# pedro-morgado/spatialaudiogen

Hardware: AMD Instinct MI355X
Metric: ambisonic seconds generated/sec (0.1 s windows, 224x448 video) (higher is better)
Workload: dtype f32 (fp32 in / out / accumulate; products on the 16-bit matrix cores with fp32-equivalent operand splits: two fp16 planes (3 products per multiply) for the ResNet trunk's 3x3 convs, whose operand ranges batch-norm bounds, three bf16 planes (6 products) elsewhere - measured against the fp64 oracle as

## Files before the change

spatialaudiogen_amd/csrc/conv3g.hip:

```cpp
#include "igemm3_common.h"

namespace sagen {

typedef _Float16 f16x8g __attribute__((ext_vector_type(8)));

constexpr int conv3g_wgs_per_cu(int BM, int BN, int KS, bool H2) {
    const int lds = 2 * KS * (BM + BN) * (H2 ? 64 : 96) + 512;
    return 3 * lds <= 160 * 1024 ? 3 : (2 * lds <= 160 * 1024 ? 2 : 1);
}

template <int BM, int BN, int WM, int WN, int KS, bool H2, int EPI = 0>
__global__ __launch_bounds__(256, conv3g_wgs_per_cu(BM, BN, KS, H2)) void conv3g_kernel(const IgemmDesc d_in) {
    IgemmDesc d = d_in;
    if (d.grp.G > 1) igemm_relocate(d, (int)blockIdx.z);
    constexpr int MT = WM / 32, NT = WN / 32;
    constexpr int WAVES_N = BN / WN, WAVES_M = BM / WM;
    static_assert(WAVES_N * WAVES_M == 4, "4 waves per workgroup");
    constexpr int NPL = H2 ? 2 : 3, SB = NPL * 32, UPS = NPL * 2;
    constexpr int NPR = H2 ? 3 : 6;
    constexpr int A_INST = BM * UPS / 64, B_INST = BN * UPS / 64;
    static_assert(BM * UPS % 64 == 0 && BN * UPS % 64 == 0, "operand images must be whole DMA instructions");
    constexpr int A_PW = (A_INST + 3) / 4, B_PW = (B_INST + 3) / 4;
    constexpr int A_BYTES = A_INST * 1024, B_BYTES = B_INST * 1024;
    constexpr int T_BYTES = A_BYTES + B_BYTES;
    constexpr int ST_BYTES = KS * T_BYTES;
    constexpr int SPT = A_PW + B_PW;
    constexpr int CNT = KS * SPT;
    constexpr int NM1 = NPR * MT * NT;
    constexpr int NMG = KS * NM1;
    static_assert(CNT <= NMG, "one DMA slot per MFMA slot at most");
    constexpr int NF = NPL * (MT + NT);
    constexpr int SMEM_BYTES = 2 * ST_BYTES;
    __shared__ __attribute__((aligned(16))) char smem[SMEM_BYTES];

    const int tid = threadIdx.x;
    const int lane = tid & 63;
    const int wave = __builtin_amdgcn_readfirstlane(tid >> 6);
    const int wm = wave / WAVES_N, wn = wave % WAVES_N;
    const int Wp = d.Win + 1;
    const int HinP = d.xp3_rows > 0 ? d.xp3_rows : d.Hin;
    const int nchunk = d.Cin >> 4;
    const int NKT = d.ntaps * nchunk;
    const int G = (NKT + KS - 1) / KS;
    const int nM = (d.M + BM - 1) / BM, nN = (d.N + BN - 1) / BN;

    const __amdgpu_buffer_rsrc_t x_rsrc = __builtin_amdgcn_make_buffer_rsrc((void*)d.xp3, 0, d.xp3_bytes, 0x00020000);
    const __amdgpu_buffer_rsrc_t w_rsrc = H2 ? __builtin_amdgcn_make_buffer_rsrc((void*)d.wh2, 0, d.wh2_bytes, 0x00020000)
                                             : __builtin_amdgcn_make_buffer_rsrc((void*)(d.w + (size_t)d.N * d.Kpad), 0, d.w_bytes / 2 * 3, 0x00020000);

    const int xcd = (blockIdx.x + blockIdx.z) & 7;
    const int per = (nM + 7) >> 3;
    const int t_run = blockIdx.x >> 3;
    const int my_tiles = max(min((xcd + 1) * per, nM) - xcd * per, 0) * nN;
    if (t_run >= my_tiles) return;
    const int tq = t_run / nN;
    const int m0 = (xcd * per + tq) * BM, n0 = (t_run - tq * nN) * BN;

    unsigned a_base[A_PW], a_bad[A_PW], a_cur[A_PW];
#pragma unroll
    for (int j = 0; j < A_PW; ++j) {
        const int inst = wave + 4 * j;
        const int U = inst * 64 + lane;
        const int slot = U / UPS, rem = U - UPS * slot;
        const int unit = H2 ? (rem ^ ((slot >> 2) & 3)) : ((rem & ~1) | ((rem & 1) ^ ((slot >> 3) & 1)));
        const int m = m0 + slot;
        a_base[j] = 0; a_bad[j] = 0xffffffffu;
        if (inst < A_INST && m < d.M) {
            const unsigned row = __umulhi((unsigned)m, d.p3_magic_wp);
            const int wo = m - (int)row * d.Wg;
            const unsigned b = __umulhi(row, d.p3_magic_h);
            const int ho = (int)row - (int)b * d.Hg;
            const int hi = (d.g_h0 + ho) * d.in_sh + d.tap_h0 - d.xp3_row0, wi = (d.g_w0 + wo) * d.in_sw + d.tap_w0;
            const int pix = ((int)b * HinP + hi) * Wp + wi;
            a_base[j] = (unsigned)(pix * SB + unit * 16);
            unsigned bad = 0;
            for (int th = 0; th * d.TW < d.ntaps; ++th) {
                const int hh = hi + th * d.tap_sh;
                if (hh < 0 || hh >= HinP) bad |= 1u << th;
            }
            a_bad[j] = bad;
        }
    }
    unsigned b_voff[B_PW];
#pragma unroll
    for (int j = 0; j < B_PW; ++j) {
        const int inst = wave + 4 * j;
        const int L = inst * 64 + lane;
        const int pl = L / (2 * BN), n = (L >> 1) % BN, half = L & 1;
        b_voff[j] = (inst < B_INST && n0 + n < d.N) ? (unsigned)((pl * d.N + n0 + n) * 32 + 16 * (half ^ ((n >> 3) & 1))) : OOB;
    }

    int q_th = 0, q_tw = 0, q_ch = 0, q_kt = 0;
    unsigned i_asoff = 0, i_bsoff = 0, i_dead = 0;
    char* i_tile = smem;
    auto begin_tile = [&](char* dst) {
        i_tile = dst;
        i_dead = q_kt >= NKT ? OOB : 0u;
        const unsigned tapd = (unsigned)((q_th * d.tap_sh * Wp + q_tw * d.tap_sw) * SB);
#pragma unroll
        for (int j = 0; j < A_PW; ++j) a_cur[j] = ((a_bad[j] >> q_th) & 1u) ? OOB : a_base[j] + tapd;
        i_asoff = (unsigned)q_ch * d.xp3_cstride;
        i_bsoff = (unsigned)q_kt * (unsigned)(d.N * SB);
        ++q_kt; ++q_ch;
        const int wrap_c = q_ch == nchunk ? 1 : 0;
        q_ch = wrap_c ? 0 : q_ch;
        q_tw += wrap_c;
        const int wrap_w = q_tw == d.TW ? 1 : 0;
        q_tw = wrap_w ? 0 : q_tw;
        q_th += wrap_w;
    };
    auto issue_one = [&](int s) {
        if (s < A_PW) {
            const int inst = wave + 4 * s;
            if (A_INST % 4 == 0 || inst < A_INST) dma16(x_rsrc, (float*)(i_tile + inst * 1024), a_cur[s] | i_dead, i_dead ? 0u : i_asoff);
        } else {
            const int j = s - A_PW;
            const int inst = wave + 4 * j;
            if (B_INST % 4 == 0 || inst < B_INST) dma16(w_rsrc, (float*)(i_tile + A_BYTES + inst * 1024), b_voff[j] | i_dead, i_dead ? 0u : i_bsoff);
        }
    };

    f32x16 acc[MT][NT];
#pragma unroll
    for (int i = 0; i < MT; ++i)
#pragma unroll
        for (int j = 0; j < NT; ++j)
#pragma unroll
            for (int e = 0; e < 16; ++e) acc[i][j][e] = 0.f;

    const int li = lane & 31, kk = lane >> 5;
    int a_foff[MT];
#pragma unroll
    for (int i = 0; i < MT; ++i) {
        const int sl = wm * WM + i * 32 + li;
        a_foff[i] = H2 ? sl * 64 + 16 * (kk ^ ((sl >> 2) & 3)) : sl * 96 + 16 * (kk ^ ((sl >> 3) & 1));
    }
    const int b_foff = A_BYTES + (wn * WN + li) * 32 + 16 * (kk ^ ((li >> 3) & 1));
    constexpr int TA[6] = {H2 ? 1 : 0, 0, H2 ? 0 : 1, 0, 2, 1}, TB[6] = {0, 1, 0, 2, 0, 1};

    int stage = 0;
#pragma unroll
    for (int ks = 0; ks < KS; ++ks) {
        begin_tile(smem + ks * T_BYTES);
#pragma unroll
        for (int s = SPT - 1; s >= 0; --s) issue_one(s);
    }

    auto group = [&](auto issue_tag) {
        constexpr bool ISSUE = decltype(issue_tag)::value;
        const char* st = smem + stage * ST_BYTES;
        char* const nst = smem + (stage ^ 1) * ST_BYTES;
        bf16x8 fq[2][NF];
        auto load_frag = [&](int buf, int ks, int f) {
            const int pl = f / (MT + NT), r = f - pl * (MT + NT);
            const char* tb = st + ks * T_BYTES;
            if (r < MT) fq[buf][f] = *reinterpret_cast<const bf16x8*>(tb + (H2 ? (a_foff[r] ^ (pl * 32)) : a_foff[r] + pl * 32));
            else fq[buf][f] = *reinterpret_cast<const bf16x8*>(tb + b_foff + pl * (BN * 32) + (r - MT) * 32 * 32);
        };
#pragma unroll
        for (int f = 0; f < NF; ++f) load_frag(0, 0, f);
#pragma unroll
        for (int ks = 0; ks < KS; ++ks) {
            const int cb = ks & 1;
#pragma unroll
            for (int tt = 0; tt < NPR; ++tt)
#pragma unroll
                for (int i = 0; i < MT; ++i)
#pragma unroll
                    for (int j = 0; j < NT; ++j) {
                        const int k = (tt * MT + i) * NT + j;
                        const int idx = ks * NM1 + k;
                        __builtin_amdgcn_sched_barrier(0);
                        if constexpr (H2)
                            acc[i][j] = __builtin_amdgcn_mfma_f32_32x32x16_f16(__builtin_bit_cast(f16x8g, fq[cb][TA[tt] * (MT + NT) + i]),
                                                                               __builtin_bit_cast(f16x8g, fq[cb][TB[tt] * (MT + NT) + MT + j]), acc[i][j], 0, 0, 0);
                        else
                            acc[i][j] = __builtin_amdgcn_mfma_f32_32x32x16_bf16(fq[cb][TA[tt] * (MT + NT) + i], fq[cb][TB[tt] * (MT + NT) + MT + j],
                                                                                acc[i][j], 0, 0, 0);
                        if (ks + 1 < KS) {
#pragma unroll
                            for (int f = 0; f < NF; ++f)
                                if (f * NM1 / NF == k) load_frag(cb ^ 1, ks + 1, f);
                        }
                        if (ISSUE && idx < CNT) {
                            const int tks = idx / SPT, s = idx - tks * SPT;
                            if (s == 0) begin_tile(nst + tks * T_BYTES);
                            issue_one(SPT - 1 - s);
                        }
                    }
        }
        __builtin_amdgcn_sched_barrier(0);
        stage ^= 1;
    };

    for (int it = 0; it + 1 < G; ++it) {
        asm volatile("s_waitcnt vmcnt(0)" ::: "memory");
        lds_barrier();
        group(std::true_type{});
    }
    asm volatile("s_waitcnt vmcnt(0)" ::: "memory");
    lds_barrier();
    group(std::false_type{});

    float osc = 1.f;
    if constexpr (H2) osc = d.h2_a_inv[0] * d.h2_w_inv[0];
    lds_barrier();
    if constexpr (EPI == 1) {
        if constexpr (H2) {
#pragma unroll
            for (int i = 0; i < MT; ++i)
#pragma unroll
                for (int j = 0; j < NT; ++j)
#pragma unroll
                    for (int e = 0; e < 16; ++e) acc[i][j][e] *= osc;
        }
        igemm_epilogue_maskmix<BM, BN, WM, WN, SMEM_BYTES / 4>(d, acc, reinterpret_cast<float*>(smem), m0, n0, tid);
        return;
    }
    {
        const int colb = n0 + wn * WN + li;
        const bool plain = d.bias == nullptr && !d.relu_out;
        const __amdgpu_buffer_rsrc_t y_rsrc = __builtin_amdgcn_make_buffer_rsrc((void*)d.y, 0, d.y_bytes, 0x00020000);
        const unsigned ldy4 = (unsigned)d.ldy * 4u;
        const int mrow = m0 + wm * WM + 4 * kk;
        const unsigned rbase = (unsigned)mrow * ldy4;
        float bias_j[NT], cs[NT], cq[NT];
        float amax = 0.f;
        unsigned col4[NT];
#pragma unroll
        for (int j = 0; j < NT; ++j) {
            const bool ok = colb + 32 * j < d.N;
            col4[j] = ok ? (unsigned)(colb + 32 * j) * 4u : OOB;
            bias_j[j] = (d.bias != nullptr && ok) ? d.bias[colb + 32 * j] : 0.f;
            cs[j] = 0.f; cq[j] = 0.f;
        }
        auto epilogue = [&](auto fast_tag) {
            constexpr bool FAST = decltype(fast_tag)::value;
#pragma unroll
            for (int i = 0; i < MT; ++i)
#pragma unroll
                for (int e = 0; e < 16; ++e) {
                    const int ro = i * 32 + (e & 3) + 8 * (e >> 2);
                    const bool ok = mrow + ro < d.M;
                    const float sc = ok ? osc : 0.f;
                    const unsigned roff = ok ? rbase + (unsigned)ro * ldy4 + (FAST ? (unsigned)(colb * 4) : 0u) : OOB;
#pragma unroll
                    for (int j = 0; j < NT; ++j) {
                        float v = acc[i][j][e] * sc;
                        if (FAST) {
                            cs[j] += v;
                            cq[j] = __builtin_fmaf(v, v, cq[j]);
                            __builtin_amdgcn_raw_buffer_store_b32(__builtin_bit_cast(unsigned, v), y_rsrc, roff, 128 * j, 0);
                        } else {
                            const unsigned off = ((roff | col4[j]) & OOB) ? OOB : roff + col4[j];
                            if (col4[j] & OOB) v = 0.f;
                            cs[j] += v;
                            cq[j] = __builtin_fmaf(v, v, cq[j]);
                            v += bias_j[j];
                            if (d.relu_out) v = fmaxf(v, 0.f);
                            amax = fmaxf(amax, (off & OOB) ? 0.f : fabsf(v));
                            __builtin_amdgcn_raw_buffer_store_b32(__builtin_bit_cast(unsigned, v), y_rsrc, off, 0, 0);
                        }
                    }
                }
        };
        if (plain && n0 + BN <= d.N && d.amax_out == nullptr) epilogue(std::true_type{});
        else epilogue(std::false_type{});
        if (d.amax_out != nullptr) igemm_publish_amax(d.amax_out, amax);
        if (d.stats != nullptr) {
            lds_barrier();
            float* const red = reinterpret_cast<float*>(smem);
            static_assert(WAVES_M * 2 * 2 * BN * 4 <= SMEM_BYTES, "statistics staging must fit the ring");
#pragma unroll
            for (int j = 0; j < NT; ++j) {
                red[((wm * 2 + kk) * 2 + 0) * BN + wn * WN + j * 32 + li] = cs[j];
                red[((wm * 2 + kk) * 2 + 1) * BN + wn * WN + j * 32 + li] = cq[j];
            }
            lds_barrier();
            for (int t = tid; t < 2 * BN; t += 256) {
                const int which = t / BN, col = t - which * BN;
                if (n0 + col < d.N) {
                    float sum = 0.f;
#pragma unroll
                    for (int g = 0; g < WAVES_M * 2; ++g) sum += red[(g * 2 + which) * BN + col];
                    atomicAdd(&d.stats[(long)which * d.N + n0 + col], (double)sum);
                }
            }
        }
    }
}

template <int BM, int BN, int WM, int WN, int KS, bool H2, int EPI = 0>
static int launch_conv3g(const IgemmDesc& d, hipStream_t s) {
    const int per = (cdiv(d.M, BM) + 7) / 8;
    const int grid = 8 * per * cdiv(d.N, BN);
    hipLaunchKernelGGL((conv3g_kernel<BM, BN, WM, WN, KS, H2, EPI>), dim3(grid, 1, d.grp.G), dim3(256), 0, s, d);
    SAGEN_LAUNCH_CHECK();
    return SAGEN_OK;
}

bool conv3g_ok(const IgemmDesc& d) {
    if (d.Cin % 16 || d.K != d.ntaps * d.Cin || d.Kpad != d.K) return false;
    if (d.ntaps < 1 || d.TW < 1 || d.ntaps % d.TW || d.ntaps / d.TW > 32) return false;
    if (d.in_scale != nullptr || d.bn_in.acc != nullptr) return false;
    if (d.mm_out != nullptr) {
        if (d.xp3_fmt != 1 || d.Cout != 32 || d.dsh * d.dsw <= 1 || d.Wg % 64 || (d.dsw * d.Cout) % 128 || d.splitk != 1 || !d.mm_coeffs) return false;
    } else {
        if (d.dsh * d.dsw != 1 || d.g_h0 != 0 || d.g_w0 != 0) return false;
        if (d.y_rstride != (long)d.Wg * d.ldy || (d.M > d.Hg * d.Wg && d.y_bstride != (long)d.Hg * d.Wg * d.ldy)) return false;
    }
    const int t_lo = std::min(0, (d.TW - 1) * d.tap_sw), t_hi = std::max(0, (d.TW - 1) * d.tap_sw);
    const int w_lo = d.g_w0 * d.in_sw + d.tap_w0 + t_lo, w_hi = (d.g_w0 + d.Wg - 1) * d.in_sw + d.tap_w0 + t_hi;
    return w_lo >= -1 && w_hi <= d.Win;
}

int conv3g_dispatch(const IgemmDesc& d_in, IgemmTile tile, hipStream_t s) {
    IgemmDesc d = d_in;
    if (!d.xp3 || d.p3_np <= 0) return fail(SAGEN_ERR_NULL, "conv3g: the P3 activation planes are missing");
    if (d.splitk != 1) return fail(SAGEN_ERR_UNSUPPORTED, "conv3g: no split-K");
    if (!conv3g_ok(d)) return fail(SAGEN_ERR_UNSUPPORTED, "conv3g: geometry not supported");
    if ((long)(d.M + 512) * d.Wg >= (1L << 32) || ((long)(d.M + 512) / d.Wg + 1) * d.Hg >= (1L << 32))
        return fail(SAGEN_ERR_UNSUPPORTED, "conv3g: too many pixels for 32-bit index arithmetic");
    if ((long)d.p3_np * 96 >= (1L << 31) || (long)d.xp3_cstride * (d.Cin / 16) >= (1L << 31) || d.xp3_bytes == 0)
        return fail(SAGEN_ERR_UNSUPPORTED, "conv3g: the activation planes exceed 2 GiB buffer addressing (use a smaller batch)");
    const bool mm = igemm_tile_traits(tile) & TF_FUSED_TAIL;
    if (mm != (d.mm_out != nullptr)) return fail(SAGEN_ERR_UNSUPPORTED, "conv3g: the fused decoder tail and the tile do not match");
    const bool h2 = igemm_tile_traits(tile) & TF_FP16X2;
    if (h2 != (d.xp3_fmt == 1)) return fail(SAGEN_ERR_UNSUPPORTED, "conv3g: the planes' format does not match the tile");
    if (h2 && (!d.wh2 || !d.h2_a_inv || !d.h2_w_inv)) return fail(SAGEN_ERR_NULL, "conv3g: the fp16x2 filter planes / scales are missing");
    if (!mm) {
        const long y_bytes = ((long)(d.M - 1) * d.ldy + d.N) * 4;
        if (y_bytes >= (1L << 31)) return fail(SAGEN_ERR_UNSUPPORTED, "conv3g: the output exceeds 2 GiB buffer addressing (use a smaller batch)");
        d.y_bytes = (unsigned)y_bytes;
    }
    d.p3_magic_wp = (unsigned)((1UL << 32) / (unsigned)d.Wg) + 1u;
    d.p3_magic_h = (unsigned)((1UL << 32) / (unsigned)d.Hg) + 1u;
#define SAGEN_TILE_HAS_P3G ,
#define SAGEN_TILE_HAS_P3GH ,
#define SAGEN_TILE_HAS_P3GH_MM ,
    switch (tile) {
        SAGEN_TILES(SAGEN_TILE_CASE)
        default: return fail(SAGEN_ERR_UNSUPPORTED, "conv3g: bad tile id %d", (int)tile);
    }
}

}
```

spatialaudiogen_amd/csrc/igemm_common.h:

```cpp
#pragma once
#include "kernels.h"
#include "h2_planes.h"

namespace sagen {

typedef float f32x16 __attribute__((ext_vector_type(16)));
constexpr int MAX_TAPS = 128;
constexpr unsigned OOB = 0x80000000u;
constexpr int MAX_BN_C = 512;

struct RowInfo {
    unsigned boff;
    unsigned nmlo, nmhi;
    int hrem, wrem;
    int pad;
    long rowoff;
};

__device__ __forceinline__ void dma16(__amdgpu_buffer_rsrc_t rsrc, float* lds, unsigned voff, unsigned soff) {
#if defined(__HIP_DEVICE_COMPILE__) && !defined(SAGEN_ABLATE_DMA)
    __builtin_amdgcn_raw_ptr_buffer_load_lds(rsrc, (__attribute__((address_space(3))) void*)lds, 16, voff, soff, 0, 0);
#endif
}

template <int N> __device__ __forceinline__ void wait_vmcnt() {
    if constexpr (N == 0) asm volatile("s_waitcnt vmcnt(0)" ::: "memory");
    else if constexpr (N == 1) asm volatile("s_waitcnt vmcnt(1)" ::: "memory");
    else if constexpr (N == 2) asm volatile("s_waitcnt vmcnt(2)" ::: "memory");
    else if constexpr (N == 3) asm volatile("s_waitcnt vmcnt(3)" ::: "memory");
    else if constexpr (N == 4) asm volatile("s_waitcnt vmcnt(4)" ::: "memory");
    else if constexpr (N == 5) asm volatile("s_waitcnt vmcnt(5)" ::: "memory");
    else if constexpr (N == 6) asm volatile("s_waitcnt vmcnt(6)" ::: "memory");
    else if constexpr (N == 7) asm volatile("s_waitcnt vmcnt(7)" ::: "memory");
    else if constexpr (N == 8) asm volatile("s_waitcnt vmcnt(8)" ::: "memory");
    else if constexpr (N == 9) asm volatile("s_waitcnt vmcnt(9)" ::: "memory");
    else asm volatile("s_waitcnt vmcnt(0)" ::: "memory");
}

__device__ __forceinline__ void lds_barrier() {
    asm volatile("s_waitcnt lgkmcnt(0)" ::: "memory");
    __builtin_amdgcn_s_barrier();
    asm volatile("" ::: "memory");
}


template <int BM>
__device__ __forceinline__ void igemm_setup(const IgemmDesc& d, int m0, int tid, bool uni, RowInfo* s_row, int* s_tapb,
                                            float (*s_bn)[MAX_BN_C]) {
    const int HgWg = d.Hg * d.Wg;
    if (!uni)
        for (int t = tid; t < d.ntaps; t += 256) {
            const int th = t / d.TW;
            s_tapb[t] = (((th * d.tap_sh + d.tap_h0) * d.Win + ((t - th * d.TW) * d.tap_sw + d.tap_w0)) * d.ldx) * 4;
        }
    for (int r = tid; r < BM; r += 256) {
        const int m = m0 + r;
        RowInfo ri;
        ri.boff = 0; ri.nmlo = 0xffffffffu; ri.nmhi = 0xffffffffu; ri.hrem = 0; ri.wrem = 0; ri.pad = 0; ri.rowoff = 0;
        if (m < d.M) {
            const int b = m / HgWg;
            const int rem = m - b * HgWg;
            const int ia = rem / d.Wg;
            const int a = d.g_h0 + ia, bb = d.g_w0 + (rem - ia * d.Wg);
            const int hi0 = a * d.in_sh, wi0 = bb * d.in_sw;
            ri.boff = (unsigned)(((long)b * d.x_bstride + ((long)hi0 * d.Win + wi0) * d.ldx) * 4);
            ri.rowoff = (long)b * d.y_bstride + (long)(a * d.dsh) * d.y_rstride + (long)(bb * d.dsw) * d.ldy;
            ri.hrem = d.Hlim - a * d.dsh;
            ri.wrem = d.Wlim - bb * d.dsw;
            if (d.no_bounds) {
                ri.nmlo = 0; ri.nmhi = 0;
            } else {
                unsigned lo = 0, hi = 0;
                for (int t = 0; t < d.ntaps; ++t) {
                    const int th = t / d.TW;
                    const int hh = hi0 + th * d.tap_sh + d.tap_h0, ww = wi0 + (t - th * d.TW) * d.tap_sw + d.tap_w0;
                    const unsigned bad = ((unsigned)hh < (unsigned)d.Hin && (unsigned)ww < (unsigned)d.Win) ? 0u : 1u;
                    if (t < 32) lo |= bad << t; else hi |= bad << (t - 32);
                }
                ri.nmlo = lo; ri.nmhi = hi;
            }
        }
        s_row[r] = ri;
    }
    if (d.bn_in.acc != nullptr) {
        for (int ch = tid; ch < d.Cin; ch += 256) {
            const double mean = d.bn_in.acc[ch] * d.bn_in.inv_count;
            double var = d.bn_in.acc[d.Cin + ch] * d.bn_in.inv_count - mean * mean;
            var = var < 0.0 ? 0.0 : var;
            const double sc = (double)d.bn_in.gamma[ch] / sqrt(var + (double)d.bn_in.eps);
            s_bn[0][ch] = (float)sc;
            s_bn[1][ch] = (float)((double)d.bn_in.beta[ch] - mean * sc);
        }
    } else if (d.in_scale != nullptr) {
        for (int ch = tid; ch < d.Cin; ch += 256) { s_bn[0][ch] = d.in_scale[ch]; s_bn[1][ch] = d.in_shift[ch]; }
    }
    __syncthreads();

}

__device__ __forceinline__ void igemm_publish_amax(float* amax_out, float v) {
    v = wave_max_f(v);
    if ((threadIdx.x & 63) == 0 && v > 0.f)
        atomicMax(reinterpret_cast<unsigned*>(amax_out) + H2_AMAX_STRIDE * ((blockIdx.x * 4 + (threadIdx.x >> 6)) & (H2_AMAX_SLOTS - 1)), __builtin_bit_cast(unsigned, v));
}

template <int BM, int BN, int WM, int WN>
__device__ __forceinline__ void igemm_epilogue(const IgemmDesc& d, f32x16 (&acc)[WM / 32][WN / 32], const RowInfo* s_row,
                                               float* red, int m0, int n0, int z, int tid) {
    constexpr int MT = WM / 32, NT = WN / 32;
    constexpr int WAVES_N = BN / WN, WAVES_M = BM / WM;
    const int lane = tid & 63;
    const int wave = __builtin_amdgcn_readfirstlane(tid >> 6);
    const int wm = wave / WAVES_N, wn = wave % WAVES_N;
    const int li = lane & 31, kk = lane >> 5;
    const int dswC = d.dsw * d.Cout;
    const bool to_ws = d.splitk_ws != nullptr;
    float csum[NT], csq[NT];
    float amax = 0.f;
#pragma unroll
    for (int j = 0; j < NT; ++j) {
        csum[j] = 0.f;
        csq[j] = 0.f;
        const int n = n0 + wn * WN + j * 32 + li;
        const bool nok = n < d.N;
        int ry = 0, rx = 0, o = n;
        if (d.dsh * d.dsw > 1) {
            ry = n / dswC;
            const int rem = n - ry * dswC;
            rx = rem / d.Cout;
            o = rem - rx * d.Cout;
        }
        const long coloff = (long)ry * d.y_rstride + (long)rx * d.ldy + o;
        const float bias = (d.bias && nok && !to_ws) ? d.bias[o] : 0.f;
#pragma unroll
        for (int i = 0; i < MT; ++i) {
#pragma unroll
            for (int e = 0; e < 16; ++e) {
                const int row = wm * WM + i * 32 + (e & 3) + 8 * (e >> 2) + 4 * kk;
                const int m = m0 + row;
                float v = acc[i][j][e];
                if (to_ws) {
                    if (nok && m < d.M) {
                        float* q = &d.splitk_ws[((long)z * d.M + m) * d.N + n];
                        if (d.sk_ticket) __hip_atomic_store(q, v, __ATOMIC_RELAXED, __HIP_MEMORY_SCOPE_AGENT);
                        else *q = v;
                    }
                } else {
                    const bool ok = nok && ry < s_row[row].hrem && rx < s_row[row].wrem;
                    if (ok) {
                        csum[j] += v;
                        csq[j] += v * v;
                        v += bias;
                        if (d.relu_out) v = fmaxf(v, 0.f);
                        d.y[s_row[row].rowoff + coloff] = v;
                        amax = fmaxf(amax, fabsf(v));
                    }
                }
            }
        }
    }
    if (d.amax_out != nullptr && !to_ws) igemm_publish_amax(d.amax_out, amax);
    if (to_ws && d.sk_ticket != nullptr) {
        __shared__ int s_last;
        asm volatile("s_waitcnt vmcnt(0)" ::: "memory");
        __syncthreads();
        const int tile = (m0 / BM) * ((d.N + BN - 1) / BN) + n0 / BN;
        if (tid == 0) {
            const int t = __hip_atomic_fetch_add(&d.sk_ticket[tile], 1, __ATOMIC_RELAXED, __HIP_MEMORY_SCOPE_AGENT);
            s_last = t == d.splitk - 1;
            if (s_last) __hip_atomic_store(&d.sk_ticket[tile], 0, __ATOMIC_RELAXED, __HIP_MEMORY_SCOPE_AGENT);
        }
        __syncthreads();
        if (s_last) {
            constexpr int C4 = BN / 4;
            auto ld4 = [](const float* q) {
                return make_float4(__hip_atomic_load(q, __ATOMIC_RELAXED, __HIP_MEMORY_SCOPE_AGENT), __hip_atomic_load(q + 1, __ATOMIC_RELAXED, __HIP_MEMORY_SCOPE_AGENT),
                                   __hip_atomic_load(q + 2, __ATOMIC_RELAXED, __HIP_MEMORY_SCOPE_AGENT), __hip_atomic_load(q + 3, __ATOMIC_RELAXED, __HIP_MEMORY_SCOPE_AGENT));
            };
            const long MN = (long)d.M * d.N;
            for (int idx = tid; idx < BM * C4; idx += 256) {
                const int r = idx / C4, m = m0 + r, n = n0 + 4 * (idx - r * C4);
                if (m >= d.M || n >= d.N) continue;
                const float* p = d.splitk_ws + (long)m * d.N + n;
                float4 v = make_float4(0.f, 0.f, 0.f, 0.f);
                int zz = 0;
                for (; zz + 4 <= d.splitk; zz += 4, p += 4 * MN) {
                    const float4 t0 = ld4(p), t1 = ld4(p + MN);
                    const float4 t2 = ld4(p + 2 * MN), t3 = ld4(p + 3 * MN);
                    v.x += (t0.x + t1.x) + (t2.x + t3.x); v.y += (t0.y + t1.y) + (t2.y + t3.y);
                    v.z += (t0.z + t1.z) + (t2.z + t3.z); v.w += (t0.w + t1.w) + (t2.w + t3.w);
                }
                for (; zz < d.splitk; ++zz, p += MN) {
                    const float4 t = ld4(p);
                    v.x += t.x; v.y += t.y; v.z += t.z; v.w += t.w;
                }
                if (d.bias) { v.x += d.bias[n]; v.y += d.bias[n + 1]; v.z += d.bias[n + 2]; v.w += d.bias[n + 3]; }
                if (d.relu_out) { v.x = fmaxf(v.x, 0.f); v.y = fmaxf(v.y, 0.f); v.z = fmaxf(v.z, 0.f); v.w = fmaxf(v.w, 0.f); }
                for (int rr = 0; rr < d.sk_rep; ++rr) *reinterpret_cast<float4*>(d.y + ((long)m * d.sk_rep + rr) * d.ldy + n) = v;
            }
        }
    }
    if (d.stats != nullptr) {
        __syncthreads();
#pragma unroll
        for (int j = 0; j < NT; ++j) {
            float s = wave_xor_add<32>(csum[j]);
            float q = wave_xor_add<32>(csq[j]);
            if (kk == 0) {
                const int col = wn * WN + j * 32 + li;
                red[(0 * WAVES_M + wm) * BN + col] = s;
                red[(1 * WAVES_M + wm) * BN + col] = q;
            }
        }
        __syncthreads();
        for (int t = tid; t < 2 * BN; t += 256) {
            const int which = t / BN, col = t - which * BN;
            const int n = n0 + col;
            if (n < d.N) {
                float s = 0.f;
#pragma unroll
                for (int w2 = 0; w2 < WAVES_M; ++w2) s += red[(which * WAVES_M + w2) * BN + col];
                atomicAdd(&d.stats[(long)which * d.N + n], (double)s);
            }
        }
    }
}

template <int BM, int BN, int WM, int WN, int CAP>
__device__ __forceinline__ bool igemm_epilogue_rows(const IgemmDesc& d, f32x16 (&acc)[WM / 32][WN / 32], const RowInfo* s_row,
                                                    float* red, int n0, int tid) {
    constexpr int MT = WM / 32, NT = WN / 32;
    constexpr int WAVES_N = BN / WN, WAVES_M = BM / WM;
    constexpr int TPR = BN / 4, RPP = 256 / TPR;
    if constexpr (WM % RPP != 0 || WM * BN + 2 * RPP * BN > CAP) {
        return false;
    } else {
        if (d.dsh * d.dsw != 1 || d.splitk_ws != nullptr) return false;
        constexpr int NPASS = WM / RPP;
        const int lane = tid & 63;
        const int wave = __builtin_amdgcn_readfirstlane(tid >> 6);
        const int wm = wave / WAVES_N, wn = wave % WAVES_N;
        const int li = lane & 31, kk = lane >> 5;
        float* const tile = red;
        float* const part_sums = red + WM * BN;
        const int c4 = tid % TPR, rg = tid / TPR;
        const int n = n0 + 4 * c4;
        const bool vec_ok = n + 3 < d.N && (d.ldy % 4 == 0) && ((reinterpret_cast<uintptr_t>(d.y) & 15) == 0);
        float4 bias = make_float4(0.f, 0.f, 0.f, 0.f);
        if (d.bias) {
            bias.x = n < d.N ? d.bias[n] : 0.f; bias.y = n + 1 < d.N ? d.bias[n + 1] : 0.f;
            bias.z = n + 2 < d.N ? d.bias[n + 2] : 0.f; bias.w = n + 3 < d.N ? d.bias[n + 3] : 0.f;
        }
        float4 cs = make_float4(0.f, 0.f, 0.f, 0.f), cq = make_float4(0.f, 0.f, 0.f, 0.f);
        float amax = 0.f;
#pragma unroll
        for (int part = 0; part < WAVES_M; ++part) {
            if (wm == part) {
#pragma unroll
                for (int i = 0; i < MT; ++i)
#pragma unroll
                    for (int j = 0; j < NT; ++j)
#pragma unroll
                        for (int e = 0; e < 16; ++e)
                            tile[(i * 32 + (e & 3) + 8 * (e >> 2) + 4 * kk) * BN + wn * WN + j * 32 + li] = acc[i][j][e];
            }
            __syncthreads();
            long ro[NPASS];
            bool ok[NPASS];
            float4 tv[NPASS];
#pragma unroll
            for (int k = 0; k < NPASS; ++k) {
                const RowInfo& ri = s_row[part * WM + rg + k * RPP];
                ok[k] = ri.hrem > 0 && ri.wrem > 0;
                ro[k] = ri.rowoff;
            }
#pragma unroll
            for (int k = 0; k < NPASS; ++k) tv[k] = *reinterpret_cast<const float4*>(tile + (rg + k * RPP) * BN + 4 * c4);
#pragma unroll
            for (int k = 0; k < NPASS; ++k) {
                if (!ok[k]) continue;
                float4 v = tv[k];
                cs.x += v.x; cs.y += v.y; cs.z += v.z; cs.w += v.w;
                cq.x += v.x * v.x; cq.y += v.y * v.y; cq.z += v.z * v.z; cq.w += v.w * v.w;
                v.x += bias.x; v.y += bias.y; v.z += bias.z; v.w += bias.w;
                if (d.relu_out) { v.x = fmaxf(v.x, 0.f); v.y = fmaxf(v.y, 0.f); v.z = fmaxf(v.z, 0.f); v.w = fmaxf(v.w, 0.f); }
                float* dst = d.y + ro[k] + n;
                if (vec_ok) *reinterpret_cast<float4*>(dst) = v;
                else {
                    if (n < d.N) dst[0] = v.x;
                    if (n + 1 < d.N) dst[1] = v.y;
                    if (n + 2 < d.N) dst[2] = v.z;
                    if (n + 3 < d.N) dst[3] = v.w;
                }
                amax = fmaxf(amax, fmaxf(fmaxf(n < d.N ? fabsf(v.x) : 0.f, n + 1 < d.N ? fabsf(v.y) : 0.f),
                                         fmaxf(n + 2 < d.N ? fabsf(v.z) : 0.f, n + 3 < d.N ? fabsf(v.w) : 0.f)));
            }
            if (part + 1 < WAVES_M) __syncthreads();
        }
        if (d.amax_out != nullptr) igemm_publish_amax(d.amax_out, amax);
        if (d.stats != nullptr) {
            *reinterpret_cast<float4*>(part_sums + (0 * RPP + rg) * BN + 4 * c4) = cs;
            *reinterpret_cast<float4*>(part_sums + (1 * RPP + rg) * BN + 4 * c4) = cq;
            __syncthreads();
            for (int t = tid; t < 2 * BN; t += 256) {
                const int which = t / BN, col = t - which * BN;
                if (n0 + col < d.N) {
                    float sum = 0.f;
#pragma unroll
                    for (int g = 0; g < RPP; ++g) sum += part_sums[(which * RPP + g) * BN + col];
                    atomicAdd(&d.stats[(long)which * d.N + n0 + col], (double)sum);
                }
            }
        }
        return true;
    }
}

template <int BM, int BN, int WM, int WN, int CAP>
__device__ __forceinline__ void igemm_epilogue_maskmix(const IgemmDesc& d, f32x16 (&acc)[WM / 32][WN / 32], float* red, int m0, int n0,
                                                       int tid) {
    constexpr int NTR = 32;
    constexpr int MT = WM / 32, NT = WN / 32;
    constexpr int WAVES_N = BN / WN, WAVES_M = BM / WM;
    constexpr int SUBS = BN / NTR, ITEMS = WM * SUBS * 2;
    static_assert(WM * BN + 7 * NTR <= CAP, "mask-mix staging must fit the tile ring");
    static_assert(ITEMS % 2 == 0 && BN % NTR == 0, "whole output pixels per tile");
    float* const tile = red;
    float* const wl = red + WM * BN;
    float* const bs = wl + 6 * NTR;
    const int lane = tid & 63;
    const int wave = __builtin_amdgcn_readfirstlane(tid >> 6);
    const int wm = wave / WAVES_N, wn = wave % WAVES_N;
    const int li = lane & 31, kk = lane >> 5;
    const int HgWg = d.Hg * d.Wg;
    const int b = m0 / HgWg;
    const int rem = m0 - b * HgWg;
    const int ia = rem / d.Wg;
    const int q0 = d.g_w0 + rem - ia * d.Wg;
    const int dswC = d.dsw * NTR;
    const int ry = n0 / dswC, rx0 = (n0 - ry * dswC) / NTR;
    const int y = (d.g_h0 + ia) * d.dsh + ry, fi = y - d.mm_row0;
    if (m0 >= d.M || y >= d.Hlim || fi < 0 || fi >= d.mm_nf) return;
    const int f = d.mm_f_lo + fi;
    const int n_lo = max(256 * f - 1216, 0), n_hi = min(256 * f - 1216 + 1023, 4799);
    const int s_lo = n_lo / 1600, s_hi = n_hi / 1600;
    const bool two = s_hi != s_lo;
    for (int i = tid; i < 6 * NTR; i += 256) {
        const int j = i % NTR, o = (i / NTR) % 3, si = i / (3 * NTR);
        wl[i] = d.mm_coeffs[(((long)b * 3 + (si ? s_hi : s_lo)) * 3 + o) * (NTR + 1) + j];
    }
    if (tid < NTR) bs[tid] = d.bias ? d.bias[tid] : 0.f;
#pragma unroll
    for (int part = 0; part < WAVES_M; ++part) {
        if (wm == part) {
#pragma unroll
            for (int i = 0; i < MT; ++i)
#pragma unroll
                for (int j = 0; j < NT; ++j)
#pragma unroll
                    for (int e = 0; e < 16; ++e)
                        tile[(i * 32 + (e & 3) + 8 * (e >> 2) + 4 * kk) * BN + wn * WN + j * 32 + li] = acc[i][j][e];
        }
        __syncthreads();
        for (int item = tid; item < ITEMS; item += 256) {
            const int half = item & 1, sub = (item >> 1) % SUBS, r = (item >> 1) / SUBS;
            float e[6] = {0.f, 0.f, 0.f, 0.f, 0.f, 0.f};
#pragma unroll
            for (int q4 = 0; q4 < 4; ++q4) {
                const float4 v = *reinterpret_cast<const float4*>(tile + r * BN + sub * NTR + half * 16 + 4 * q4);
                const float vv[4] = {v.x, v.y, v.z, v.w};
#pragma unroll
                for (int u = 0; u < 4; ++u) {
                    const int j = half * 16 + 4 * q4 + u;
                    const float sg = __builtin_amdgcn_rcpf(1.f + __builtin_amdgcn_exp2f(-1.4426950408889634f * (vv[u] + bs[j])));
#pragma unroll
                    for (int o = 0; o < 3; ++o) {
                        e[o] = fmaf(wl[o * NTR + j], sg, e[o]);
                        if (two) e[3 + o] = fmaf(wl[(3 + o) * NTR + j], sg, e[3 + o]);
                    }
                }
            }
#pragma unroll
            for (int c = 0; c < 6; ++c) e[c] = wave_xor_add<1>(e[c]);
            const int row = part * WM + r;
            const int x = (q0 + row) * d.dsw + rx0 + sub;
            if (half == 0 && m0 + row < d.M && x < d.Wlim) {
                float4* dst = reinterpret_cast<float4*>(d.mm_out + (((long)b * d.mm_nf + fi) * d.Wlim + x) * 8);
                dst[0] = make_float4(e[0], e[1], e[2], e[3]);
                dst[1] = make_float4(e[4], e[5], 0.f, 0.f);
            }
        }
        if (part + 1 < WAVES_M) __syncthreads();
    }
}

}
```

Before: 3203.

## Fuse mask-mix epilogue into registers with swapped MFMA operands and permuted weight rows

```diff
diff --git a/spatialaudiogen_amd/csrc/conv3g.hip b/spatialaudiogen_amd/csrc/conv3g.hip
--- a/spatialaudiogen_amd/csrc/conv3g.hip
+++ b/spatialaudiogen_amd/csrc/conv3g.hip
@@ -4,13 +4,13 @@
 
 typedef _Float16 f16x8g __attribute__((ext_vector_type(8)));
 
-constexpr int conv3g_wgs_per_cu(int BM, int BN, int KS, bool H2) {
-    const int lds = 2 * KS * (BM + BN) * (H2 ? 64 : 96) + 512;
+constexpr int conv3g_wgs_per_cu(int BM, int BN, int KS, bool H2, int EPI = 0) {
+    const int lds = 2 * KS * (BM + BN) * (H2 ? 64 : 96) + 512 + (EPI == 1 ? 4 * MM_WAVE_FLOATS * 4 : 0);
     return 3 * lds <= 160 * 1024 ? 3 : (2 * lds <= 160 * 1024 ? 2 : 1);
 }
 
 template <int BM, int BN, int WM, int WN, int KS, bool H2, int EPI = 0>
-__global__ __launch_bounds__(256, conv3g_wgs_per_cu(BM, BN, KS, H2)) void conv3g_kernel(const IgemmDesc d_in) {
+__global__ __launch_bounds__(256, conv3g_wgs_per_cu(BM, BN, KS, H2, EPI)) void conv3g_kernel(const IgemmDesc d_in) {
     IgemmDesc d = d_in;
     if (d.grp.G > 1) igemm_relocate(d, (int)blockIdx.z);
     constexpr int MT = WM / 32, NT = WN / 32;
@@ -30,7 +30,8 @@
     constexpr int NMG = KS * NM1;
     static_assert(CNT <= NMG, "one DMA slot per MFMA slot at most");
     constexpr int NF = NPL * (MT + NT);
-    constexpr int SMEM_BYTES = 2 * ST_BYTES;
+    constexpr int RING_BYTES = 2 * ST_BYTES;
+    constexpr int SMEM_BYTES = RING_BYTES + (EPI == 1 ? 4 * MM_WAVE_FLOATS * 4 : 0);
     __shared__ __attribute__((aligned(16))) char smem[SMEM_BYTES];
 
     const int tid = threadIdx.x;
@@ -87,7 +88,16 @@
         const int inst = wave + 4 * j;
         const int L = inst * 64 + lane;
         const int pl = L / (2 * BN), n = (L >> 1) % BN, half = L & 1;
-        b_voff[j] = (inst < B_INST && n0 + n < d.N) ? (unsigned)((pl * d.N + n0 + n) * 32 + 16 * (half ^ ((n >> 3) & 1))) : OOB;
+        const int ns = EPI == 1 ? (n & ~31) | mm_track_of_row(n & 31) : n;
+        b_voff[j] = (inst < B_INST && n0 + n < d.N) ? (unsigned)((pl * d.N + n0 + ns) * 32 + 16 * (half ^ ((n >> 3) & 1))) : OOB;
+    }
+    MaskTail mm_tail;
+    float mm_wv[4];
+    float* const mm_wl = reinterpret_cast<float*>(smem + RING_BYTES) + wave * MM_WAVE_FLOATS;
+    float mm_osc = 1.f;
+    if constexpr (EPI == 1) {
+        mm_tail = igemm_maskmix_stage(d, mm_wv, m0, n0, lane);
+        mm_osc = d.h2_a_inv[0] * d.h2_w_inv[0];
     }
 
     int q_th = 0, q_tw = 0, q_ch = 0, q_kt = 0;
@@ -145,6 +155,7 @@
 #pragma unroll
         for (int s = SPT - 1; s >= 0; --s) issue_one(s);
     }
+    if constexpr (EPI == 1) igemm_maskmix_put(mm_wl, mm_wv, lane);
 
     auto group = [&](auto issue_tag) {
         constexpr bool ISSUE = decltype(issue_tag)::value;
@@ -171,7 +182,10 @@
                         const int k = (tt * MT + i) * NT + j;
                         const int idx = ks * NM1 + k;
                         __builtin_amdgcn_sched_barrier(0);
-                        if constexpr (H2)
+                        if constexpr (H2 && EPI == 1)
+                            acc[i][j] = __builtin_amdgcn_mfma_f32_32x32x16_f16(__builtin_bit_cast(f16x8g, fq[cb][TB[tt] * (MT + NT) + MT + j]),
+                                                                               __builtin_bit_cast(f16x8g, fq[cb][TA[tt] * (MT + NT) + i]), acc[i][j], 0, 0, 0);
+                        else if constexpr (H2)
                             acc[i][j] = __builtin_amdgcn_mfma_f32_32x32x16_f16(__builtin_bit_cast(f16x8g, fq[cb][TA[tt] * (MT + NT) + i]),
                                                                                __builtin_bit_cast(f16x8g, fq[cb][TB[tt] * (MT + NT) + MT + j]), acc[i][j], 0, 0, 0);
                         else
@@ -202,21 +216,14 @@
     lds_barrier();
     group(std::false_type{});
 
+    if constexpr (EPI == 1) {
+        static_assert(H2, "the fused tail contracts fp16x2 planes");
+        igemm_epilogue_maskmix_regs<BM, BN, WM, WN>(d, acc, mm_osc, mm_tail, mm_wl, m0, tid);
+        return;
+    }
     float osc = 1.f;
     if constexpr (H2) osc = d.h2_a_inv[0] * d.h2_w_inv[0];
     lds_barrier();
-    if constexpr (EPI == 1) {
-        if constexpr (H2) {
-#pragma unroll
-            for (int i = 0; i < MT; ++i)
-#pragma unroll
-                for (int j = 0; j < NT; ++j)
-#pragma unroll
-                    for (int e = 0; e < 16; ++e) acc[i][j][e] *= osc;
-        }
-        igemm_epilogue_maskmix<BM, BN, WM, WN, SMEM_BYTES / 4>(d, acc, reinterpret_cast<float*>(smem), m0, n0, tid);
-        return;
-    }
     {
         const int colb = n0 + wn * WN + li;
         const bool plain = d.bias == nullptr && !d.relu_out;
diff --git a/spatialaudiogen_amd/csrc/igemm_common.h b/spatialaudiogen_amd/csrc/igemm_common.h
--- a/spatialaudiogen_amd/csrc/igemm_common.h
+++ b/spatialaudiogen_amd/csrc/igemm_common.h
@@ -394,4 +394,122 @@
     }
 }
 
-}
+constexpr int MM_NTR = 32;
+constexpr int MM_WAVE_FLOATS = 7 * MM_NTR;
+
+__device__ __forceinline__ constexpr int mm_track_of_row(int r) { return (r & 3) | ((r >> 1) & 12) | ((r << 2) & 16); }
+
+struct MaskTail {
+    int b, fi, q0, rx0;
+    bool live, two;
+};
+
+__device__ __forceinline__ MaskTail igemm_maskmix_stage(const IgemmDesc& d, float (&wv)[4], int m0, int n0, int lane) {
+    MaskTail g;
+    const int HgWg = d.Hg * d.Wg;
+    g.b = m0 / HgWg;
+    const int rem = m0 - g.b * HgWg;
+    const int ia = rem / d.Wg;
+    g.q0 = d.g_w0 + rem - ia * d.Wg;
+    const int dswC = d.dsw * MM_NTR;
+    const int ry = n0 / dswC;
+    g.rx0 = (n0 - ry * dswC) / MM_NTR;
+    const int y = (d.g_h0 + ia) * d.dsh + ry;
+    g.fi = y - d.mm_row0;
+    g.live = !(m0 >= d.M || y >= d.Hlim || g.fi < 0 || g.fi >= d.mm_nf);
+    g.two = false;
+    wv[0] = wv[1] = wv[2] = wv[3] = 0.f;
+    if (g.live) {
+        const int f = d.mm_f_lo + g.fi;
+        const int n_lo = max(256 * f - 1216, 0), n_hi = min(256 * f - 1216 + 1023, 4799);
+        const int s_lo = n_lo / 1600, s_hi = n_hi / 1600;
+        g.two = s_hi != s_lo;
+#pragma unroll
+        for (int k = 0; k < 3; ++k) {
+            const int i = lane + 64 * k;
+            const int j = i % MM_NTR, o = (i / MM_NTR) % 3, si = i / (3 * MM_NTR);
+            wv[k] = d.mm_coeffs[(((long)g.b * 3 + (si ? s_hi : s_lo)) * 3 + o) * (MM_NTR + 1) + j];
+        }
+        if (d.bias) wv[3] = d.bias[lane & (MM_NTR - 1)];
+    }
+    return g;
+}
+
+__device__ __forceinline__ void igemm_maskmix_put(float* wl, const float (&wv)[4], int lane) {
+#pragma unroll
+    for (int k = 0; k < 3; ++k) wl[lane + 64 * k] = wv[k];
+    if (lane < MM_NTR) wl[6 * MM_NTR + lane] = wv[3];
+}
+
+template <int BM, int BN, int WM, int WN>
+__device__ __forceinline__ void igemm_epilogue_maskmix_regs(const IgemmDesc& d, f32x16 (&acc)[WM / 32][WN / 32], float osc, const MaskTail& g,
+                                                            const float* wl, int m0, int tid) {
+    constexpr int MT = WM / 32, NT = WN / 32;
+    constexpr int WAVES_N = BN / WN;
+    static_assert(NT % 2 == 0, "the half-waves store the sub-positions of a pair");
+    if (!g.live) return;
+    const int lane = tid & 63;
+    const int wave = __builtin_amdgcn_readfirstlane(tid >> 6);
+    const int wm = wave / WAVES_N, wn = wave % WAVES_N;
+    const int li = lane & 31, kk = lane >> 5;
+    const float4* const wq = reinterpret_cast<const float4*>(wl + 16 * kk);
+    auto row16 = [&](int r, float (&w)[16]) {
+#pragma unroll
+        for (int q = 0; q < 4; ++q) {
+            const float4 v = wq[r * (MM_NTR / 4) + q];
+            w[4 * q] = v.x; w[4 * q + 1] = v.y; w[4 * q + 2] = v.z; w[4 * q + 3] = v.w;
+        }
+    };
+    {
+        float bs[16];
+        row16(6, bs);
+#pragma unroll
+        for (int i = 0; i < MT; ++i)
+#pragma unroll
+            for (int j = 0; j < NT; ++j)
+#pragma unroll
+                for (int e = 0; e < 16; ++e)
+                    acc[i][j][e] = __builtin_amdgcn_rcpf(1.f + __builtin_amdgcn_exp2f(-1.4426950408889634f * __builtin_fmaf(acc[i][j][e], osc, bs[e])));
+    }
+    float s[MT][NT][6];
+#pragma unroll
+    for (int i = 0; i < MT; ++i)
+#pragma unroll
+        for (int j = 0; j < NT; ++j)
+#pragma unroll
+            for (int c = 0; c < 6; ++c) s[i][j][c] = 0.f;
+    auto sums = [&](int c) {
+        float w[16];
+        row16(c, w);
+#pragma unroll
+        for (int i = 0; i < MT; ++i)
+#pragma unroll
+            for (int j = 0; j < NT; ++j)
+#pragma unroll
+                for (int e = 0; e < 16; ++e) s[i][j][c] = __builtin_fmaf(w[e], acc[i][j][e], s[i][j][c]);
+    };
+    sums(0); sums(1); sums(2);
+    if (g.two) { sums(3); sums(4); sums(5); }
+    float* const out = d.mm_out + ((long)g.b * d.mm_nf + g.fi) * d.Wlim * 8;
+#pragma unroll
+    for (int i = 0; i < MT; ++i)
+#pragma unroll
+        for (int p = 0; p < NT / 2; ++p) {
+            float t[6];
+#pragma unroll
+            for (int c = 0; c < 6; ++c) {
+                float lo = s[i][2 * p][c], hi = s[i][2 * p + 1][c];
+                asm volatile("s_nop 1\n\tv_permlane32_swap_b32 %0, %1" : "+v"(lo), "+v"(hi));
+                t[c] = lo + hi;
+            }
+            const int row = wm * WM + i * 32 + li;
+            const int x = (g.q0 + row) * d.dsw + g.rx0 + wn * NT + 2 * p + kk;
+            if (m0 + row < d.M && x < d.Wlim) {
+                float4* dst = reinterpret_cast<float4*>(out + (long)x * 8);
+                dst[0] = make_float4(t[0], t[1], t[2], t[3]);
+                dst[1] = make_float4(t[4], t[5], 0.f, 0.f);
+            }
+        }
+}
+
+}
```

After: 3220, median of 6. Within noise of the previous version (+0.5%).
